# eps696/aphantasia

Measured on NVIDIA H100. Metric: optimization steps/sec @1280x720 FFT, 200 samples, ViT-B/32, higher is better.
Workload: dtype bf16

## Files before the change

aphantasia_b200/csrc/tc_gemm.cuh:

```cuda
#pragma once
#include "aph_common.cuh"
#include <cuda.h>

namespace aph {

typedef __nv_bfloat16 bf16;

struct GemmEpi {
  const float* bias = nullptr;
  const float* resid = nullptr;
  const bf16* gelu_in = nullptr;
  float* out_f32 = nullptr;
  bf16* out_bf16 = nullptr;
  bf16* out_pre = nullptr;
  int act = 0;
  int unpatch_p = 0;
  int unpatch_g = 0;
  int ld_resid = 0;
  int ld_out = 0;
};

struct GemmShape { int M, N, K; };

constexpr int GEMM_BM = 128;
constexpr int GEMM_BK = 64;
constexpr int GEMM_UK = 16;
constexpr int GEMM_THREADS = 3 * 128;

enum : int {
  EPI_F32 = 0,
  EPI_BF16 = 1,
  EPI_BIAS_BF16 = 2,
  EPI_BIAS_GELU = 3,
  EPI_BIAS_RESID = 4,
  EPI_GELUGRAD_BF16 = 5,
  EPI_UNPATCH = 6,
  EPI_KINDS = 7
};

__device__ __forceinline__ uint32_t smem_u32(const void* p) { return (uint32_t)__cvta_generic_to_shared(p); }

__device__ __forceinline__ void mbar_init(uint64_t* bar, uint32_t count) {
  asm volatile("mbarrier.init.shared::cta.b64 [%0], %1;" ::"r"(smem_u32(bar)), "r"(count));
}
__device__ __forceinline__ void mbar_expect_tx(uint64_t* bar, uint32_t bytes) {
  asm volatile("mbarrier.arrive.expect_tx.shared::cta.b64 _, [%0], %1;" ::"r"(smem_u32(bar)), "r"(bytes) : "memory");
}
__device__ __forceinline__ void mbar_arrive(uint64_t* bar) {
  asm volatile("mbarrier.arrive.shared::cta.b64 _, [%0];" ::"r"(smem_u32(bar)) : "memory");
}
__device__ __forceinline__ void mbar_wait(uint64_t* bar, uint32_t parity) {
  uint32_t done;
  do {
    asm volatile(
        "{\n\t.reg .pred p;\n\t"
        "mbarrier.try_wait.parity.shared::cta.b64 p, [%1], %2;\n\t"
        "selp.u32 %0, 1, 0, p;\n\t}"
        : "=r"(done) : "r"(smem_u32(bar)), "r"(parity) : "memory");
  } while (!done);
}
__device__ __forceinline__ void fence_barrier_init() { asm volatile("fence.mbarrier_init.release.cluster;" ::: "memory"); }

__device__ __forceinline__ void tma_prefetch_desc(const CUtensorMap* m) {
  asm volatile("prefetch.tensormap [%0];" ::"l"(reinterpret_cast<uint64_t>(m)) : "memory");
}
__device__ __forceinline__ void tma_load_2d(void* dst, const CUtensorMap* m, uint64_t* bar, int x, int y) {
  asm volatile("cp.async.bulk.tensor.2d.shared::cluster.global.mbarrier::complete_tx::bytes [%0], [%1, {%3, %4}], [%2];"
               ::"r"(smem_u32(dst)), "l"(reinterpret_cast<uint64_t>(m)), "r"(smem_u32(bar)), "r"(x), "r"(y) : "memory");
}
__device__ __forceinline__ void tma_load_3d(uint32_t dst_saddr, const CUtensorMap* m, uint64_t* bar, int x, int y, int z) {
  asm volatile("cp.async.bulk.tensor.3d.shared::cluster.global.mbarrier::complete_tx::bytes [%0], [%1, {%3, %4, %5}], [%2];"
               ::"r"(dst_saddr), "l"(reinterpret_cast<uint64_t>(m)), "r"(smem_u32(bar)), "r"(x), "r"(y), "r"(z) : "memory");
}
__device__ __forceinline__ void tma_load_2d_hint(void* dst, const CUtensorMap* m, uint64_t* bar, int x, int y, uint64_t policy) {
  asm volatile("cp.async.bulk.tensor.2d.shared::cluster.global.mbarrier::complete_tx::bytes.L2::cache_hint [%0], [%1, {%3, %4}], [%2], %5;"
               ::"r"(smem_u32(dst)), "l"(reinterpret_cast<uint64_t>(m)), "r"(smem_u32(bar)), "r"(x), "r"(y), "l"(policy) : "memory");
}
__device__ __forceinline__ uint64_t l2_policy_evict_last() {
  uint64_t p;
  asm volatile("createpolicy.fractional.L2::evict_last.b64 %0, 1.0;" : "=l"(p));
  return p;
}

__device__ __forceinline__ uint64_t make_smem_desc(uint32_t saddr) {
  uint64_t d = 0;
  d |= (uint64_t)((saddr & 0x3FFFF) >> 4);
  d |= (uint64_t)1 << 16;
  d |= (uint64_t)(1024 >> 4) << 32;
  d |= (uint64_t)1 << 62;
  return d;
}
__device__ __forceinline__ void wgmma_fence() { asm volatile("wgmma.fence.sync.aligned;" ::: "memory"); }
__device__ __forceinline__ void wgmma_commit() { asm volatile("wgmma.commit_group.sync.aligned;" ::: "memory"); }
template <int N> __device__ __forceinline__ void wgmma_wait() { asm volatile("wgmma.wait_group.sync.aligned %0;" ::"n"(N) : "memory"); }
template <int R> __device__ __forceinline__ void setmaxnreg_inc() { asm volatile("setmaxnreg.inc.sync.aligned.u32 %0;" ::"n"(R)); }
template <int R> __device__ __forceinline__ void setmaxnreg_dec() { asm volatile("setmaxnreg.dec.sync.aligned.u32 %0;" ::"n"(R)); }

template <int BN> struct Wgmma;
#define APH_WG_REGS8(o) "+f"(d[o]), "+f"(d[o + 1]), "+f"(d[o + 2]), "+f"(d[o + 3]), "+f"(d[o + 4]), "+f"(d[o + 5]), "+f"(d[o + 6]), "+f"(d[o + 7])
template <> struct Wgmma<128> {
  static __device__ __forceinline__ void mma(float (&d)[64], uint64_t da, uint64_t db, int acc) {
    asm volatile(
        "{\n\t.reg .pred p;\n\tsetp.ne.b32 p, %66, 0;\n\t"
        "wgmma.mma_async.sync.aligned.m64n128k16.f32.bf16.bf16 "
        "{%0, %1, %2, %3, %4, %5, %6, %7, %8, %9, %10, %11, %12, %13, %14, %15, %16, %17, %18, %19, %20, %21, %22, %23, "
        "%24, %25, %26, %27, %28, %29, %30, %31, %32, %33, %34, %35, %36, %37, %38, %39, %40, %41, %42, %43, %44, %45, %46, %47, "
        "%48, %49, %50, %51, %52, %53, %54, %55, %56, %57, %58, %59, %60, %61, %62, %63}, %64, %65, p, 1, 1, 0, 0;\n\t}"
        : APH_WG_REGS8(0), APH_WG_REGS8(8), APH_WG_REGS8(16), APH_WG_REGS8(24), APH_WG_REGS8(32), APH_WG_REGS8(40), APH_WG_REGS8(48), APH_WG_REGS8(56)
        : "l"(da), "l"(db), "r"(acc));
  }
};
template <> struct Wgmma<256> {
  static __device__ __forceinline__ void mma(float (&d)[128], uint64_t da, uint64_t db, int acc) {
    asm volatile(
        "{\n\t.reg .pred p;\n\tsetp.ne.b32 p, %130, 0;\n\t"
        "wgmma.mma_async.sync.aligned.m64n256k16.f32.bf16.bf16 "
        "{%0, %1, %2, %3, %4, %5, %6, %7, %8, %9, %10, %11, %12, %13, %14, %15, %16, %17, %18, %19, %20, %21, %22, %23, "
        "%24, %25, %26, %27, %28, %29, %30, %31, %32, %33, %34, %35, %36, %37, %38, %39, %40, %41, %42, %43, %44, %45, %46, %47, "
        "%48, %49, %50, %51, %52, %53, %54, %55, %56, %57, %58, %59, %60, %61, %62, %63, %64, %65, %66, %67, %68, %69, %70, %71, "
        "%72, %73, %74, %75, %76, %77, %78, %79, %80, %81, %82, %83, %84, %85, %86, %87, %88, %89, %90, %91, %92, %93, %94, %95, "
        "%96, %97, %98, %99, %100, %101, %102, %103, %104, %105, %106, %107, %108, %109, %110, %111, %112, %113, %114, %115, "
        "%116, %117, %118, %119, %120, %121, %122, %123, %124, %125, %126, %127}, %128, %129, p, 1, 1, 0, 0;\n\t}"
        : APH_WG_REGS8(0), APH_WG_REGS8(8), APH_WG_REGS8(16), APH_WG_REGS8(24), APH_WG_REGS8(32), APH_WG_REGS8(40), APH_WG_REGS8(48), APH_WG_REGS8(56),
          APH_WG_REGS8(64), APH_WG_REGS8(72), APH_WG_REGS8(80), APH_WG_REGS8(88), APH_WG_REGS8(96), APH_WG_REGS8(104), APH_WG_REGS8(112), APH_WG_REGS8(120)
        : "l"(da), "l"(db), "r"(acc));
  }
};
#undef APH_WG_REGS8

__device__ __forceinline__ float sigmoid1702(float x) {
  float t;
  asm("tanh.approx.f32 %0, %1;" : "=f"(t) : "f"(0.851f * x));
  return fmaf(0.5f, t, 0.5f);
}
__device__ __forceinline__ float quickgelu(float x) { return x * sigmoid1702(x); }
__device__ __forceinline__ float quickgelu_grad(float x) {
  const float s = sigmoid1702(x);
  return s * (1.f + 1.702f * x * (1.f - s));
}
__device__ __forceinline__ uint32_t pack_bf16(float lo, float hi) {
  __nv_bfloat162 v = __floats2bfloat162_rn(lo, hi);
  return *reinterpret_cast<uint32_t*>(&v);
}

template <int BN>
struct GemmCfg {
  static constexpr int A_BYTES = GEMM_BM * GEMM_BK * 2;
  static constexpr int B_BYTES = BN * GEMM_BK * 2;
  static constexpr int STAGE_BYTES = A_BYTES + B_BYTES;
  static constexpr int STAGES = (BN == 256) ? 4 : 6;
  static constexpr int BAR_OFFSET = STAGES * STAGE_BYTES;
  static constexpr int SMEM = BAR_OFFSET + 2 * STAGES * 8 + 1024;
};

__device__ __forceinline__ void consumer_bar_sync(int id) { asm volatile("bar.sync %0, 256;" ::"r"(id) : "memory"); }
__device__ __forceinline__ void consumer_bar_arrive(int id) { asm volatile("bar.arrive %0, 256;" ::"r"(id) : "memory"); }

template <int EPI>
constexpr bool epi_bf16_out() { return EPI == EPI_BF16 || EPI == EPI_BIAS_BF16 || EPI == EPI_BIAS_GELU || EPI == EPI_GELUGRAD_BF16; }

template <int EPI>
__device__ __forceinline__ void epi_store2(const GemmEpi& epi, size_t out_row, size_t res_row, int row, int col, float v0, float v1,
                                           float2 bb) {
  const size_t off = out_row + col;
  if (EPI == EPI_F32) {
    *reinterpret_cast<float2*>(epi.out_f32 + off) = make_float2(v0, v1);
  } else if (EPI == EPI_BIAS_RESID) {
    const float2 r = __ldg(reinterpret_cast<const float2*>(epi.resid + res_row + col));
    *reinterpret_cast<float2*>(epi.out_f32 + off) = make_float2(v0 + bb.x + r.x, v1 + bb.y + r.y);
  } else {
    const int p = epi.unpatch_p, g = epi.unpatch_g, R = p * g;
    const int ch = col / (p * p), rem = col - ch * p * p, py = rem / p, px = rem - py * p;
    const int s = row / (g * g), pr = row - s * g * g, gy = pr / g, gx = pr - gy * g;
    *reinterpret_cast<float2*>(epi.out_f32 + (((size_t)s * 3 + ch) * R + gy * p + py) * R + gx * p + px) = make_float2(v0, v1);
  }
}

__device__ __forceinline__ void st_global_16(void* p, const uint32_t (&w)[4]) {
  asm volatile("st.global.v4.b32 [%0], {%1, %2, %3, %4};" ::"l"(p), "r"(w[0]), "r"(w[1]), "r"(w[2]), "r"(w[3]) : "memory");
}

__device__ __forceinline__ void quad_transpose(uint32_t (&w)[4], int q) {
  const bool b0 = q & 1, b1 = q & 2;
#pragma unroll
  for (int p = 0; p < 2; ++p) {
    const uint32_t r = __shfl_xor_sync(0xffffffffu, b0 ? w[2 * p] : w[2 * p + 1], 1);
    if (b0) w[2 * p] = r; else w[2 * p + 1] = r;
  }
#pragma unroll
  for (int p = 0; p < 2; ++p) {
    const uint32_t r = __shfl_xor_sync(0xffffffffu, b1 ? w[p] : w[p + 2], 2);
    if (b1) w[p] = r; else w[p + 2] = r;
  }
}

template <int EPI>
__device__ __forceinline__ void epi_store_bf16x32(const GemmEpi& epi, int row, bool valid, int col0, int q, const float* v,
                                                  const float2* bb) {
  const size_t off = (size_t)row * epi.ld_out + col0 + 8 * q;
  uint32_t w[4], w2[4];
  if constexpr (EPI == EPI_GELUGRAD_BF16) {
    uint4 g = make_uint4(0u, 0u, 0u, 0u);
    if (valid) g = __ldg(reinterpret_cast<const uint4*>(epi.gelu_in + off));
    w2[0] = g.x; w2[1] = g.y; w2[2] = g.z; w2[3] = g.w;
    quad_transpose(w2, q);
  }
#pragma unroll
  for (int t = 0; t < 4; ++t) {
    float v0 = v[2 * t], v1 = v[2 * t + 1];
    if (EPI == EPI_BF16) {
      w[t] = pack_bf16(v0, v1);
    } else if (EPI == EPI_BIAS_BF16) {
      w[t] = pack_bf16(v0 + bb[t].x, v1 + bb[t].y);
    } else if (EPI == EPI_BIAS_GELU) {
      v0 += bb[t].x; v1 += bb[t].y;
      w2[t] = pack_bf16(v0, v1);
      w[t] = pack_bf16(quickgelu(v0), quickgelu(v1));
    } else {
      const float2 h = __bfloat1622float2(*reinterpret_cast<const __nv_bfloat162*>(&w2[t]));
      w[t] = pack_bf16(v0 * quickgelu_grad(h.x), v1 * quickgelu_grad(h.y));
    }
  }
  quad_transpose(w, q);
  if (valid) st_global_16(epi.out_bf16 + off, w);
  if constexpr (EPI == EPI_BIAS_GELU) {
    quad_transpose(w2, q);
    if (valid) st_global_16(epi.out_pre + off, w2);
  }
}

template <int BN, bool PINGPONG, int EPI>
__global__ void __launch_bounds__(GEMM_THREADS, 1)
k_gemm_bf16_tn(const __grid_constant__ CUtensorMap map_a, const __grid_constant__ CUtensorMap map_b, GemmShape shp, GemmEpi epi) {
  static_assert(BN == 128 || !PINGPONG, "the ping-pong schedule runs 128 x 128 tiles");
  using L = GemmCfg<BN>;
  constexpr int STAGES = L::STAGES;
  constexpr int MMAS = PINGPONG ? 2 : 1;
  constexpr bool HAS_BIAS = (EPI == EPI_BIAS_BF16 || EPI == EPI_BIAS_GELU || EPI == EPI_BIAS_RESID);
  pdl_trigger();
  extern __shared__ uint8_t smem_raw[];
  uint8_t* smem = reinterpret_cast<uint8_t*>((reinterpret_cast<uintptr_t>(smem_raw) + 1023) & ~(uintptr_t)1023);
  uint64_t* full_bar = reinterpret_cast<uint64_t*>(smem + L::BAR_OFFSET);
  uint64_t* empty_bar = full_bar + STAGES;

  const int wg = threadIdx.x >> 7, tid = threadIdx.x & 127;
  const int m_tiles = (shp.M + GEMM_BM - 1) / GEMM_BM, n_tiles = shp.N / BN;
  const int num_tiles = m_tiles * n_tiles, k_blocks = shp.K / GEMM_BK;

  if (threadIdx.x == 0) {
    tma_prefetch_desc(&map_a); tma_prefetch_desc(&map_b);
    for (int i = 0; i < STAGES; ++i) { mbar_init(&full_bar[i], 1); mbar_init(&empty_bar[i], PINGPONG ? 1 : 2); }
    fence_barrier_init();
  }
  __syncthreads();
  pdl_wait();

  if (wg == 0) {
    setmaxnreg_dec<40>();
    if (tid == 0) {
      const uint64_t pol_b = l2_policy_evict_last();
      uint32_t it = 0;
      for (int tile = blockIdx.x; tile < num_tiles; tile += gridDim.x) {
        const int m_blk = tile / n_tiles, n_blk = tile - m_blk * n_tiles;
        for (int kb = 0; kb < k_blocks; ++kb, ++it) {
          const uint32_t s = it % STAGES, ph = (it / STAGES) & 1;
          mbar_wait(&empty_bar[s], ph ^ 1);
          uint8_t* sa = smem + s * L::STAGE_BYTES;
          mbar_expect_tx(&full_bar[s], L::STAGE_BYTES);
          tma_load_2d(sa, &map_a, &full_bar[s], kb * GEMM_BK, m_blk * GEMM_BM);
          tma_load_2d_hint(sa + L::A_BYTES, &map_b, &full_bar[s], kb * GEMM_BK, n_blk * BN, pol_b);
        }
      }
    }
  } else {
    setmaxnreg_inc<232>();
    const int c = wg - 1, warp = tid >> 5, lane = tid & 31;
    const int row_in_tile = (PINGPONG ? 0 : 64 * c) + 16 * warp + (lane >> 2), col_in_tile = 2 * (lane & 3);
    uint32_t it = PINGPONG ? c * k_blocks : 0;
    const int tile_step = (PINGPONG ? 2 : 1) * gridDim.x;
    for (int tile = blockIdx.x + (PINGPONG ? c * gridDim.x : 0); tile / n_tiles * GEMM_BM < shp.M; tile += tile_step) {
      if (PINGPONG && tile != (int)blockIdx.x) consumer_bar_sync(1 + c);
      float d[MMAS][BN / 2];
#pragma unroll
      for (int h = 0; h < MMAS; ++h)
#pragma unroll
        for (int r = 0; r < BN / 2; ++r) d[h][r] = 0.f;
      for (int kb = 0; kb < k_blocks; ++kb, ++it) {
        const uint32_t s = it % STAGES, ph = (it / STAGES) & 1;
        mbar_wait(&full_bar[s], ph);
        const uint64_t ds = make_smem_desc(smem_u32(smem + s * L::STAGE_BYTES));
        wgmma_fence();
#pragma unroll
        for (int k = 0; k < GEMM_BK / GEMM_UK; ++k)
#pragma unroll
          for (int h = 0; h < MMAS; ++h)
            Wgmma<BN>::mma(d[h], ds + (uint64_t)((PINGPONG ? h : c) * 512 + 2 * k), ds + (uint64_t)(L::A_BYTES / 16 + 2 * k), (kb | k) != 0);
        wgmma_commit();
        wgmma_wait<1>();
        if (kb > 0 && tid == 0) mbar_arrive(&empty_bar[(it - 1) % STAGES]);
      }
      if (PINGPONG && (tile + (int)gridDim.x) / n_tiles * GEMM_BM < shp.M) consumer_bar_arrive(1 + (c ^ 1));
      wgmma_wait<0>();
      if (tid == 0) mbar_arrive(&empty_bar[(it - 1) % STAGES]);
      if (PINGPONG) it += k_blocks;
      const int m_blk = tile / n_tiles, n_blk = tile - m_blk * n_tiles;
#pragma unroll
      for (int h = 0; h < MMAS; ++h) {
        const int row0 = m_blk * GEMM_BM + 64 * h + row_in_tile, row1 = row0 + 8;
        if constexpr (epi_bf16_out<EPI>()) {
#pragma unroll
          for (int j0 = 0; j0 < BN / 8; j0 += 4) {
            const int col0 = n_blk * BN + 8 * j0;
            float2 bb[4];
            float v0[8], v1[8];
#pragma unroll
            for (int t = 0; t < 4; ++t) {
              bb[t] = HAS_BIAS ? __ldg(reinterpret_cast<const float2*>(epi.bias + col0 + 8 * t + col_in_tile)) : make_float2(0.f, 0.f);
              v0[2 * t] = d[h][4 * (j0 + t)]; v0[2 * t + 1] = d[h][4 * (j0 + t) + 1];
              v1[2 * t] = d[h][4 * (j0 + t) + 2]; v1[2 * t + 1] = d[h][4 * (j0 + t) + 3];
            }
            epi_store_bf16x32<EPI>(epi, row0, row0 < shp.M, col0, lane & 3, v0, bb);
            epi_store_bf16x32<EPI>(epi, row1, row1 < shp.M, col0, lane & 3, v1, bb);
          }
        } else {
          const size_t out0 = (size_t)row0 * epi.ld_out, out1 = out0 + 8 * (size_t)epi.ld_out;
          const size_t res0 = (EPI == EPI_BIAS_RESID) ? (size_t)row0 * epi.ld_resid : 0, res1 = res0 + 8 * (size_t)epi.ld_resid;
#pragma unroll
          for (int j = 0; j < BN / 8; ++j) {
            const int col = n_blk * BN + 8 * j + col_in_tile;
            const float2 bb = HAS_BIAS ? __ldg(reinterpret_cast<const float2*>(epi.bias + col)) : make_float2(0.f, 0.f);
            if (row0 < shp.M) epi_store2<EPI>(epi, out0, res0, row0, col, d[h][4 * j], d[h][4 * j + 1], bb);
            if (row1 < shp.M) epi_store2<EPI>(epi, out1, res1, row1, col, d[h][4 * j + 2], d[h][4 * j + 3], bb);
          }
        }
      }
    }
  }
}

int make_tmap_bf16(CUtensorMap* out, const void* base, int rows, int K, int box_rows, int64_t row_stride = 0);
int make_tmap_bf16_tokens(CUtensorMap* out, const void* base, int cols, int T, int S, int box_rows);
int launch_gemm(const void* A, const void* B, GemmShape shp, const GemmEpi& epi, cudaStream_t st, int lda = 0);

}
```

aphantasia_b200/csrc/vit_gemm.cu:

```cuda
#include "tc_gemm.cuh"
#include <atomic>
#include <mutex>
#include <vector>
#include <utility>

namespace aph {

typedef CUresult (*EncodeTiledFn)(CUtensorMap*, CUtensorMapDataType, cuuint32_t, void*, const cuuint64_t*, const cuuint64_t*,
                                  const cuuint32_t*, const cuuint32_t*, CUtensorMapInterleave, CUtensorMapSwizzle,
                                  CUtensorMapL2promotion, CUtensorMapFloatOOBfill);

static EncodeTiledFn get_encode() {
  static EncodeTiledFn fn = nullptr;
  static std::once_flag once;
  std::call_once(once, [] {
    void* p = nullptr;
    cudaDriverEntryPointQueryResult q;
    if (cudaGetDriverEntryPoint("cuTensorMapEncodeTiled", &p, cudaEnableDefault, &q) == cudaSuccess && q == cudaDriverEntryPointSuccess)
      fn = reinterpret_cast<EncodeTiledFn>(p);
  });
  return fn;
}

int make_tmap_bf16(CUtensorMap* out, const void* base, int rows, int K, int box_rows, int64_t row_stride) {
  EncodeTiledFn enc = get_encode();
  APH_REQUIRE(enc != nullptr, "cuTensorMapEncodeTiled not available from the driver");
  if (row_stride == 0) row_stride = K;
  APH_REQUIRE(row_stride >= K, "tensor map: row stride %lld < K=%d", (long long)row_stride, K);
  APH_REQUIRE((reinterpret_cast<uintptr_t>(base) & 15) == 0 && row_stride % 8 == 0, "tensor map: base/stride not 16-byte aligned");
  const cuuint64_t gdim[2] = {(cuuint64_t)K, (cuuint64_t)rows};
  const cuuint64_t gstride[1] = {(cuuint64_t)row_stride * 2};
  const cuuint32_t box[2] = {(cuuint32_t)GEMM_BK, (cuuint32_t)box_rows};
  const cuuint32_t estr[2] = {1, 1};
  const CUresult r = enc(out, CU_TENSOR_MAP_DATA_TYPE_BFLOAT16, 2, const_cast<void*>(base), gdim, gstride, box, estr,
                         CU_TENSOR_MAP_INTERLEAVE_NONE, CU_TENSOR_MAP_SWIZZLE_128B, CU_TENSOR_MAP_L2_PROMOTION_L2_256B,
                         CU_TENSOR_MAP_FLOAT_OOB_FILL_NONE);
  APH_REQUIRE(r == CUDA_SUCCESS, "cuTensorMapEncodeTiled failed: CUresult %d (rows=%d K=%d box_rows=%d)", (int)r, rows, K, box_rows);
  return 0;
}

int make_tmap_bf16_tokens(CUtensorMap* out, const void* base, int cols, int T, int S, int box_rows) {
  EncodeTiledFn enc = get_encode();
  APH_REQUIRE(enc != nullptr, "cuTensorMapEncodeTiled not available from the driver");
  APH_REQUIRE((reinterpret_cast<uintptr_t>(base) & 15) == 0 && cols % 8 == 0, "tensor map: base/stride not 16-byte aligned");
  const cuuint64_t gdim[3] = {(cuuint64_t)cols, (cuuint64_t)T, (cuuint64_t)S};
  const cuuint64_t gstride[2] = {(cuuint64_t)cols * 2, (cuuint64_t)T * cols * 2};
  const cuuint32_t box[3] = {64u, (cuuint32_t)box_rows, 1u};
  const cuuint32_t estr[3] = {1, 1, 1};
  const CUresult r = enc(out, CU_TENSOR_MAP_DATA_TYPE_BFLOAT16, 3, const_cast<void*>(base), gdim, gstride, box, estr,
                         CU_TENSOR_MAP_INTERLEAVE_NONE, CU_TENSOR_MAP_SWIZZLE_128B, CU_TENSOR_MAP_L2_PROMOTION_L2_256B,
                         CU_TENSOR_MAP_FLOAT_OOB_FILL_NONE);
  APH_REQUIRE(r == CUDA_SUCCESS, "cuTensorMapEncodeTiled (tokens) failed: CUresult %d (cols=%d T=%d S=%d box_rows=%d)", (int)r, cols, T, S, box_rows);
  return 0;
}

static bool g_prof = false;
bool gemm_profiling_on() { return g_prof; }
static std::vector<std::pair<cudaEvent_t, cudaEvent_t>> g_prof_ev;
static std::vector<double> g_prof_flops;

static std::atomic<long long> g_variant_launches[2][EPI_KINDS];

template <int BN, bool PINGPONG, int EPI>
static int launch_cfg(const void* A, const void* B, GemmShape shp, const GemmEpi& epi, cudaStream_t st, int lda) {
  using L = GemmCfg<BN>;
  static_assert(L::SMEM <= 227 * 1024, "GEMM shared-memory budget");
  g_variant_launches[(PINGPONG || BN == 256) ? 1 : 0][EPI].fetch_add(1, std::memory_order_relaxed);
  static bool configured = false;
  if (!configured) {
    APH_CUDA_OK(cudaFuncSetAttribute(k_gemm_bf16_tn<BN, PINGPONG, EPI>, cudaFuncAttributeMaxDynamicSharedMemorySize, L::SMEM));
    configured = true;
  }
  CUtensorMap ma, mb;
  if (int e = make_tmap_bf16(&ma, A, shp.M, shp.K, GEMM_BM, lda)) return e;
  if (int e = make_tmap_bf16(&mb, B, shp.N, shp.K, BN)) return e;
  const int tiles = ((shp.M + GEMM_BM - 1) / GEMM_BM) * (shp.N / BN);
  const int grid = tiles < num_sms() ? tiles : num_sms();
  cudaEvent_t e0 = nullptr, e1 = nullptr;
  if (g_prof) { cudaEventCreate(&e0); cudaEventCreate(&e1); cudaEventRecord(e0, st); }
  APH_CUDA_OK(launch_k(k_gemm_bf16_tn<BN, PINGPONG, EPI>, dim3(grid), dim3(GEMM_THREADS), (size_t)L::SMEM, st, 1, ma, mb, shp, epi));
  APH_LAUNCH_OK();
  if (g_prof) { cudaEventRecord(e1, st); g_prof_ev.emplace_back(e0, e1); g_prof_flops.push_back(2.0 * shp.M * shp.N * shp.K); }
  return 0;
}

int launch_gemm(const void* A, const void* B, GemmShape shp, const GemmEpi& epi_in, cudaStream_t st, int lda) {
  APH_REQUIRE(A && B && shp.M > 0, "gemm: null operand or empty M");
  APH_REQUIRE(shp.K % GEMM_BK == 0 && shp.K > 0, "gemm: K=%d must be a positive multiple of %d", shp.K, GEMM_BK);
  APH_REQUIRE(shp.N % 128 == 0 && shp.N > 0, "gemm: N=%d must be a positive multiple of 128", shp.N);
  APH_REQUIRE(lda == 0 || lda >= shp.K, "gemm: lda=%d < K=%d", lda, shp.K);
  APH_REQUIRE((epi_in.ld_out == 0 || epi_in.ld_out >= shp.N) && (epi_in.ld_resid == 0 || epi_in.ld_resid >= shp.N),
              "gemm: output / residual row stride below N=%d", shp.N);
  GemmEpi epi = epi_in;
  if (epi.ld_out == 0) epi.ld_out = shp.N;
  if (epi.ld_resid == 0) epi.ld_resid = shp.N;
  int kind = -1;
  const bool b = epi.bias, r = epi.resid, gi = epi.gelu_in, f = epi.out_f32, h = epi.out_bf16, pre = epi.out_pre, act = epi.act == 1, un = epi.unpatch_p > 0;
  APH_REQUIRE(!un || epi.ld_out == shp.N, "gemm: the un-patchify store takes no output stride");
  if (un && f && !b && !r && !gi && !h && !pre && !act) kind = EPI_UNPATCH;
  else if (f && !h && !b && !r && !gi && !pre && !act) kind = EPI_F32;
  else if (h && !f && !b && !r && !gi && !pre && !act) kind = EPI_BF16;
  else if (h && !f && b && !r && !gi && !pre && !act) kind = EPI_BIAS_BF16;
  else if (h && !f && b && !r && !gi && pre && act) kind = EPI_BIAS_GELU;
  else if (f && !h && b && r && !gi && !pre && !act) kind = EPI_BIAS_RESID;
  else if (h && !f && !b && !r && gi && !pre && !act) kind = EPI_GELUGRAD_BF16;
  APH_REQUIRE(kind >= 0, "gemm: unsupported epilogue combination");
  const uintptr_t bf16_ptrs = reinterpret_cast<uintptr_t>(epi.out_bf16) | reinterpret_cast<uintptr_t>(epi.out_pre) | reinterpret_cast<uintptr_t>(epi.gelu_in);
  APH_REQUIRE((bf16_ptrs & 15) == 0 && ((size_t)epi.ld_out * (f ? 4 : 2)) % 16 == 0 && ((size_t)epi.ld_resid * 4) % 16 == 0 &&
              ((size_t)lda * 2) % 16 == 0,
              "gemm: bf16 epilogue operands and row strides must be 16-byte aligned (8 columns are stored per lane)");
  const int m_tiles = (shp.M + GEMM_BM - 1) / GEMM_BM;
  const bool pingpong = m_tiles * (shp.N / 128) >= 2 * num_sms() && shp.K <= 1024;
  const bool wide = !pingpong && shp.N % 256 == 0 && m_tiles * (shp.N / 256) >= num_sms();
#define APH_GEMM_CASE(K) case K: return pingpong ? launch_cfg<128, true, K>(A, B, shp, epi, st, lda) \
                                                 : wide ? launch_cfg<256, false, K>(A, B, shp, epi, st, lda) : launch_cfg<128, false, K>(A, B, shp, epi, st, lda);
  switch (kind) {
    APH_GEMM_CASE(EPI_F32) APH_GEMM_CASE(EPI_BF16) APH_GEMM_CASE(EPI_BIAS_BF16) APH_GEMM_CASE(EPI_BIAS_GELU)
    APH_GEMM_CASE(EPI_BIAS_RESID) APH_GEMM_CASE(EPI_GELUGRAD_BF16) APH_GEMM_CASE(EPI_UNPATCH)
  }
#undef APH_GEMM_CASE
  return 2;
}

}

using namespace aph;

extern "C" int aph_gemm_bf16_tn(const void* A, const void* B, float* C, int M, int N, int K, void* stream) {
  APH_REQUIRE(C != nullptr, "aph_gemm_bf16_tn: null output");
  GemmEpi epi;
  epi.out_f32 = C;
  return launch_gemm(A, B, GemmShape{M, N, K}, epi, (cudaStream_t)stream);
}

extern "C" int aph_gemm_epi_test(const void* A, const void* B, int M, int N, int K, const float* bias, const float* resid,
                                 const void* gelu_in, int act, float* out_f32, void* out_bf16, void* out_pre,
                                 int unpatch_p, int unpatch_g, void* stream) {
  GemmEpi epi;
  epi.bias = bias; epi.resid = resid; epi.gelu_in = reinterpret_cast<const bf16*>(gelu_in); epi.act = act;
  epi.out_f32 = out_f32; epi.out_bf16 = reinterpret_cast<bf16*>(out_bf16); epi.out_pre = reinterpret_cast<bf16*>(out_pre);
  epi.unpatch_p = unpatch_p; epi.unpatch_g = unpatch_g;
  return launch_gemm(A, B, GemmShape{M, N, K}, epi, (cudaStream_t)stream);
}

extern "C" int aph_gemm_epi_strided_test(const void* A, int lda, const void* B, int M, int N, int K, const float* bias,
                                         const float* resid, int ld_resid, const void* gelu_in, int act, float* out_f32,
                                         void* out_bf16, void* out_pre, int ld_out, void* stream) {
  GemmEpi epi;
  epi.bias = bias; epi.resid = resid; epi.gelu_in = reinterpret_cast<const bf16*>(gelu_in); epi.act = act;
  epi.out_f32 = out_f32; epi.out_bf16 = reinterpret_cast<bf16*>(out_bf16); epi.out_pre = reinterpret_cast<bf16*>(out_pre);
  epi.ld_resid = ld_resid; epi.ld_out = ld_out;
  return launch_gemm(A, B, GemmShape{M, N, K}, epi, (cudaStream_t)stream, lda);
}

extern "C" int64_t aph_gemm_variant_launches(int variant, int epi) {
  if (variant < 0 || variant > 1 || epi >= EPI_KINDS) return -1;
  long long n = 0;
  for (int k = 0; k < EPI_KINDS; ++k) if (epi < 0 || epi == k) n += g_variant_launches[variant][k].load();
  return (int64_t)n;
}

extern "C" int aph_prof_gemm(int enable, double* total_ms, double* total_flops, int* launches) {
  if (enable) { g_prof = true; g_prof_ev.clear(); g_prof_flops.clear(); return 0; }
  g_prof = false;
  double ms = 0., fl = 0.;
  for (size_t i = 0; i < g_prof_ev.size(); ++i) {
    APH_CUDA_OK(cudaEventSynchronize(g_prof_ev[i].second));
    float t = 0.f;
    APH_CUDA_OK(cudaEventElapsedTime(&t, g_prof_ev[i].first, g_prof_ev[i].second));
    ms += t; fl += g_prof_flops[i];
    cudaEventDestroy(g_prof_ev[i].first); cudaEventDestroy(g_prof_ev[i].second);
  }
  if (total_ms) *total_ms = ms;
  if (total_flops) *total_flops = fl;
  if (launches) *launches = (int)g_prof_ev.size();
  g_prof_ev.clear(); g_prof_flops.clear();
  return 0;
}
```

Before: 83.68.

## Stream residual and GELU-grad epilogue operands through TMA slabs in shared memory

For the bias+residual and GELU-gradient epilogues, the GEMM now has producer threads TMA-load the residual or GELU input into a ring of 128B-swizzled shared-memory slabs. Consumers combine those slabs with the accumulators in place, and the results are written back with TMA bulk stores. This replaces per-thread scattered global loads and stores in the epilogue with bulk asynchronous transfers that can overlap the mainloop. In exchange it takes one pipeline stage away from the mainloop to make room for the slabs, and it adds mbarrier and bulk-group synchronisation per slab.

```diff
diff --git a/aphantasia_b200/csrc/tc_gemm.cuh b/aphantasia_b200/csrc/tc_gemm.cuh
--- a/aphantasia_b200/csrc/tc_gemm.cuh
+++ b/aphantasia_b200/csrc/tc_gemm.cuh
@@ -76,6 +76,14 @@
   asm volatile("cp.async.bulk.tensor.2d.shared::cluster.global.mbarrier::complete_tx::bytes.L2::cache_hint [%0], [%1, {%3, %4}], [%2], %5;"
                ::"r"(smem_u32(dst)), "l"(reinterpret_cast<uint64_t>(m)), "r"(smem_u32(bar)), "r"(x), "r"(y), "l"(policy) : "memory");
 }
+__device__ __forceinline__ void tma_store_2d(const CUtensorMap* m, const void* src, int x, int y) {
+  asm volatile("cp.async.bulk.tensor.2d.global.shared::cta.bulk_group [%0, {%2, %3}], [%1];"
+               ::"l"(reinterpret_cast<uint64_t>(m)), "r"(smem_u32(src)), "r"(x), "r"(y) : "memory");
+}
+__device__ __forceinline__ void bulk_commit() { asm volatile("cp.async.bulk.commit_group;" ::: "memory"); }
+template <int N> __device__ __forceinline__ void bulk_wait_read() { asm volatile("cp.async.bulk.wait_group.read %0;" ::"n"(N) : "memory"); }
+__device__ __forceinline__ void bulk_wait_all() { asm volatile("cp.async.bulk.wait_group 0;" ::: "memory"); }
+__device__ __forceinline__ void fence_proxy_async_smem() { asm volatile("fence.proxy.async.shared::cta;" ::: "memory"); }
 __device__ __forceinline__ uint64_t l2_policy_evict_last() {
   uint64_t p;
   asm volatile("createpolicy.fractional.L2::evict_last.b64 %0, 1.0;" : "=l"(p));
@@ -143,31 +151,36 @@
   return *reinterpret_cast<uint32_t*>(&v);
 }
 
-template <int BN>
+template <int EPI>
+constexpr bool epi_tma() { return EPI == EPI_BIAS_RESID || EPI == EPI_GELUGRAD_BF16; }
+
+template <int BN, int EPI>
 struct GemmCfg {
   static constexpr int A_BYTES = GEMM_BM * GEMM_BK * 2;
   static constexpr int B_BYTES = BN * GEMM_BK * 2;
   static constexpr int STAGE_BYTES = A_BYTES + B_BYTES;
-  static constexpr int STAGES = (BN == 256) ? 4 : 6;
-  static constexpr int BAR_OFFSET = STAGES * STAGE_BYTES;
-  static constexpr int SMEM = BAR_OFFSET + 2 * STAGES * 8 + 1024;
+  static constexpr bool TMA_EPI = epi_tma<EPI>();
+  static constexpr int STAGES = TMA_EPI ? (BN == 256 ? 3 : 5) : (BN == 256 ? 4 : 6);
+  static constexpr int SLAB_BYTES = 64 * 128;
+  static constexpr int SLAB_COLS = (EPI == EPI_BIAS_RESID) ? 32 : 64;
+  static constexpr int SLABS = TMA_EPI ? (BN == 256 ? 5 : 4) : 0;
+  static constexpr int SLAB_OFFSET = STAGES * STAGE_BYTES;
+  static constexpr int BAR_OFFSET = SLAB_OFFSET + 2 * SLABS * SLAB_BYTES;
+  static constexpr int SMEM = BAR_OFFSET + 2 * STAGES * 8 + 4 * SLABS * 8 + 1024;
 };
 
 __device__ __forceinline__ void consumer_bar_sync(int id) { asm volatile("bar.sync %0, 256;" ::"r"(id) : "memory"); }
 __device__ __forceinline__ void consumer_bar_arrive(int id) { asm volatile("bar.arrive %0, 256;" ::"r"(id) : "memory"); }
+__device__ __forceinline__ void wg_bar_sync(int id) { asm volatile("bar.sync %0, 128;" ::"r"(id) : "memory"); }
 
 template <int EPI>
-constexpr bool epi_bf16_out() { return EPI == EPI_BF16 || EPI == EPI_BIAS_BF16 || EPI == EPI_BIAS_GELU || EPI == EPI_GELUGRAD_BF16; }
+constexpr bool epi_bf16_out() { return EPI == EPI_BF16 || EPI == EPI_BIAS_BF16 || EPI == EPI_BIAS_GELU; }
 
 template <int EPI>
-__device__ __forceinline__ void epi_store2(const GemmEpi& epi, size_t out_row, size_t res_row, int row, int col, float v0, float v1,
-                                           float2 bb) {
+__device__ __forceinline__ void epi_store2(const GemmEpi& epi, size_t out_row, int row, int col, float v0, float v1) {
   const size_t off = out_row + col;
   if (EPI == EPI_F32) {
     *reinterpret_cast<float2*>(epi.out_f32 + off) = make_float2(v0, v1);
-  } else if (EPI == EPI_BIAS_RESID) {
-    const float2 r = __ldg(reinterpret_cast<const float2*>(epi.resid + res_row + col));
-    *reinterpret_cast<float2*>(epi.out_f32 + off) = make_float2(v0 + bb.x + r.x, v1 + bb.y + r.y);
   } else {
     const int p = epi.unpatch_p, g = epi.unpatch_g, R = p * g;
     const int ch = col / (p * p), rem = col - ch * p * p, py = rem / p, px = rem - py * p;
@@ -199,12 +212,6 @@
                                                   const float2* bb) {
   const size_t off = (size_t)row * epi.ld_out + col0 + 8 * q;
   uint32_t w[4], w2[4];
-  if constexpr (EPI == EPI_GELUGRAD_BF16) {
-    uint4 g = make_uint4(0u, 0u, 0u, 0u);
-    if (valid) g = __ldg(reinterpret_cast<const uint4*>(epi.gelu_in + off));
-    w2[0] = g.x; w2[1] = g.y; w2[2] = g.z; w2[3] = g.w;
-    quad_transpose(w2, q);
-  }
 #pragma unroll
   for (int t = 0; t < 4; ++t) {
     float v0 = v[2 * t], v1 = v[2 * t + 1];
@@ -212,13 +219,10 @@
       w[t] = pack_bf16(v0, v1);
     } else if (EPI == EPI_BIAS_BF16) {
       w[t] = pack_bf16(v0 + bb[t].x, v1 + bb[t].y);
-    } else if (EPI == EPI_BIAS_GELU) {
+    } else {
       v0 += bb[t].x; v1 += bb[t].y;
       w2[t] = pack_bf16(v0, v1);
       w[t] = pack_bf16(quickgelu(v0), quickgelu(v1));
-    } else {
-      const float2 h = __bfloat1622float2(*reinterpret_cast<const __nv_bfloat162*>(&w2[t]));
-      w[t] = pack_bf16(v0 * quickgelu_grad(h.x), v1 * quickgelu_grad(h.y));
     }
   }
   quad_transpose(w, q);
@@ -229,12 +233,57 @@
   }
 }
 
+__device__ __forceinline__ int swz128(int r, int k) { return r * 128 + ((k ^ (r & 7)) << 4); }
+
+__device__ __forceinline__ float2 lds_f2(uint32_t a) {
+  float2 v;
+  asm volatile("ld.shared.v2.f32 {%0, %1}, [%2];" : "=f"(v.x), "=f"(v.y) : "r"(a) : "memory");
+  return v;
+}
+__device__ __forceinline__ void sts_f2(uint32_t a, float2 v) { asm volatile("st.shared.v2.f32 [%0], {%1, %2};" ::"r"(a), "f"(v.x), "f"(v.y) : "memory"); }
+__device__ __forceinline__ uint32_t lds_u32(uint32_t a) {
+  uint32_t v;
+  asm volatile("ld.shared.b32 %0, [%1];" : "=r"(v) : "r"(a) : "memory");
+  return v;
+}
+__device__ __forceinline__ void sts_u32(uint32_t a, uint32_t v) { asm volatile("st.shared.b32 [%0], %1;" ::"r"(a), "r"(v) : "memory"); }
+__device__ __forceinline__ float2 bf16x2_to_float2(uint32_t w) { return __bfloat1622float2(*reinterpret_cast<const __nv_bfloat162*>(&w)); }
+
+template <int EPI, int NACC>
+__device__ __forceinline__ void epi_slab(uint32_t slab, const float (&v)[NACC], int g0, int rs, int q, const float* bias_cols) {
+  if constexpr (EPI == EPI_BIAS_RESID) {
+    const bool odd = rs & 1;
+#pragma unroll
+    for (int t = 0; t < 4; ++t) {
+      const int g = t ^ (odd ? 2 : 0);
+      const int a = 4 * (g0 + t), b = 4 * (g0 + (t ^ 2));
+      const float a0 = odd ? v[b] : v[a], a1 = odd ? v[b + 1] : v[a + 1];
+      const float a2 = odd ? v[b + 2] : v[a + 2], a3 = odd ? v[b + 3] : v[a + 3];
+      const float2 bb = __ldg(reinterpret_cast<const float2*>(bias_cols + 8 * g + 2 * q));
+      const uint32_t p0 = slab + swz128(rs, 2 * g + (q >> 1)) + 8 * (q & 1), p1 = slab + swz128(rs + 8, 2 * g + (q >> 1)) + 8 * (q & 1);
+      const float2 r0 = lds_f2(p0), r1 = lds_f2(p1);
+      sts_f2(p0, make_float2(a0 + bb.x + r0.x, a1 + bb.y + r0.y));
+      sts_f2(p1, make_float2(a2 + bb.x + r1.x, a3 + bb.y + r1.y));
+    }
+  } else {
+#pragma unroll
+    for (int t = 0; t < 8; ++t) {
+      const int a = 4 * (g0 + t);
+      const uint32_t p0 = slab + swz128(rs, t) + 4 * q, p1 = slab + swz128(rs + 8, t) + 4 * q;
+      const float2 h0 = bf16x2_to_float2(lds_u32(p0)), h1 = bf16x2_to_float2(lds_u32(p1));
+      sts_u32(p0, pack_bf16(v[a] * quickgelu_grad(h0.x), v[a + 1] * quickgelu_grad(h0.y)));
+      sts_u32(p1, pack_bf16(v[a + 2] * quickgelu_grad(h1.x), v[a + 3] * quickgelu_grad(h1.y)));
+    }
+  }
+}
+
 template <int BN, bool PINGPONG, int EPI>
 __global__ void __launch_bounds__(GEMM_THREADS, 1)
-k_gemm_bf16_tn(const __grid_constant__ CUtensorMap map_a, const __grid_constant__ CUtensorMap map_b, GemmShape shp, GemmEpi epi) {
+k_gemm_bf16_tn(const __grid_constant__ CUtensorMap map_a, const __grid_constant__ CUtensorMap map_b, GemmShape shp, GemmEpi epi,
+               const __grid_constant__ CUtensorMap map_ei, const __grid_constant__ CUtensorMap map_eo) {
   static_assert(BN == 128 || !PINGPONG, "the ping-pong schedule runs 128 x 128 tiles");
-  using L = GemmCfg<BN>;
-  constexpr int STAGES = L::STAGES;
+  using L = GemmCfg<BN, EPI>;
+  constexpr int STAGES = L::STAGES, SLABS = L::SLABS;
   constexpr int MMAS = PINGPONG ? 2 : 1;
   constexpr bool HAS_BIAS = (EPI == EPI_BIAS_BF16 || EPI == EPI_BIAS_GELU || EPI == EPI_BIAS_RESID);
   pdl_trigger();
@@ -242,6 +291,8 @@
   uint8_t* smem = reinterpret_cast<uint8_t*>((reinterpret_cast<uintptr_t>(smem_raw) + 1023) & ~(uintptr_t)1023);
   uint64_t* full_bar = reinterpret_cast<uint64_t*>(smem + L::BAR_OFFSET);
   uint64_t* empty_bar = full_bar + STAGES;
+  uint64_t* slab_full = empty_bar + STAGES;
+  uint64_t* slab_empty = slab_full + 2 * SLABS;
 
   const int wg = threadIdx.x >> 7, tid = threadIdx.x & 127;
   const int m_tiles = (shp.M + GEMM_BM - 1) / GEMM_BM, n_tiles = shp.N / BN;
@@ -249,7 +300,9 @@
 
   if (threadIdx.x == 0) {
     tma_prefetch_desc(&map_a); tma_prefetch_desc(&map_b);
+    if constexpr (SLABS > 0) { tma_prefetch_desc(&map_ei); tma_prefetch_desc(&map_eo); }
     for (int i = 0; i < STAGES; ++i) { mbar_init(&full_bar[i], 1); mbar_init(&empty_bar[i], PINGPONG ? 1 : 2); }
+    for (int i = 0; i < 2 * SLABS; ++i) { mbar_init(&slab_full[i], 1); mbar_init(&slab_empty[i], 1); }
     fence_barrier_init();
   }
   __syncthreads();
@@ -257,6 +310,22 @@
 
   if (wg == 0) {
     setmaxnreg_dec<40>();
+    if constexpr (SLABS > 0) if (tid == 32 || tid == 64) {
+      const int r = (tid >> 5) - 1;
+      uint8_t* ring = smem + L::SLAB_OFFSET + r * SLABS * L::SLAB_BYTES;
+      uint32_t sit = 0;
+      for (int tile = blockIdx.x + (PINGPONG ? r * gridDim.x : 0); tile < num_tiles; tile += (PINGPONG ? 2 : 1) * gridDim.x) {
+        const int m_blk = tile / n_tiles, n_blk = tile - m_blk * n_tiles;
+        for (int h = 0; h < MMAS; ++h)
+          for (int j = 0; j < BN / L::SLAB_COLS; ++j, ++sit) {
+            const uint32_t s = sit % SLABS, ph = (sit / SLABS) & 1;
+            mbar_wait(&slab_empty[r * SLABS + s], ph ^ 1);
+            mbar_expect_tx(&slab_full[r * SLABS + s], L::SLAB_BYTES);
+            tma_load_2d(ring + s * L::SLAB_BYTES, &map_ei, &slab_full[r * SLABS + s], n_blk * BN + j * L::SLAB_COLS,
+                        m_blk * GEMM_BM + 64 * (PINGPONG ? h : r));
+          }
+      }
+    }
     if (tid == 0) {
       const uint64_t pol_b = l2_policy_evict_last();
       uint32_t it = 0;
@@ -277,6 +346,7 @@
     const int c = wg - 1, warp = tid >> 5, lane = tid & 31;
     const int row_in_tile = (PINGPONG ? 0 : 64 * c) + 16 * warp + (lane >> 2), col_in_tile = 2 * (lane & 3);
     uint32_t it = PINGPONG ? c * k_blocks : 0;
+    [[maybe_unused]] uint32_t sit = 0;
     const int tile_step = (PINGPONG ? 2 : 1) * gridDim.x;
     for (int tile = blockIdx.x + (PINGPONG ? c * gridDim.x : 0); tile / n_tiles * GEMM_BM < shp.M; tile += tile_step) {
       if (PINGPONG && tile != (int)blockIdx.x) consumer_bar_sync(1 + c);
@@ -304,37 +374,65 @@
       if (tid == 0) mbar_arrive(&empty_bar[(it - 1) % STAGES]);
       if (PINGPONG) it += k_blocks;
       const int m_blk = tile / n_tiles, n_blk = tile - m_blk * n_tiles;
-#pragma unroll
-      for (int h = 0; h < MMAS; ++h) {
-        const int row0 = m_blk * GEMM_BM + 64 * h + row_in_tile, row1 = row0 + 8;
-        if constexpr (epi_bf16_out<EPI>()) {
-#pragma unroll
-          for (int j0 = 0; j0 < BN / 8; j0 += 4) {
-            const int col0 = n_blk * BN + 8 * j0;
-            float2 bb[4];
-            float v0[8], v1[8];
-#pragma unroll
-            for (int t = 0; t < 4; ++t) {
-              bb[t] = HAS_BIAS ? __ldg(reinterpret_cast<const float2*>(epi.bias + col0 + 8 * t + col_in_tile)) : make_float2(0.f, 0.f);
-              v0[2 * t] = d[h][4 * (j0 + t)]; v0[2 * t + 1] = d[h][4 * (j0 + t) + 1];
-              v1[2 * t] = d[h][4 * (j0 + t) + 2]; v1[2 * t + 1] = d[h][4 * (j0 + t) + 3];
+      if constexpr (SLABS > 0) {
+        uint8_t* ring = smem + L::SLAB_OFFSET + c * SLABS * L::SLAB_BYTES;
+        const int rs = 16 * warp + (lane >> 2), q = lane & 3;
+#pragma unroll
+        for (int h = 0; h < MMAS; ++h) {
+#pragma unroll
+          for (int j = 0; j < BN / L::SLAB_COLS; ++j, ++sit) {
+            const uint32_t s = sit % SLABS;
+            uint8_t* slab = ring + s * L::SLAB_BYTES;
+            mbar_wait(&slab_full[c * SLABS + s], (sit / SLABS) & 1);
+            epi_slab<EPI>(smem_u32(slab), d[h], j * L::SLAB_COLS / 8, rs, q, HAS_BIAS ? epi.bias + n_blk * BN + j * L::SLAB_COLS : nullptr);
+            fence_proxy_async_smem();
+            wg_bar_sync(3 + c);
+            if (tid == 0) {
+              tma_store_2d(&map_eo, slab, n_blk * BN + j * L::SLAB_COLS, m_blk * GEMM_BM + 64 * (PINGPONG ? h : c));
+              bulk_commit();
+              if (h > 0 || j > 0) {
+                bulk_wait_read<1>();
+                mbar_arrive(&slab_empty[c * SLABS + (sit - 1) % SLABS]);
+              }
             }
-            epi_store_bf16x32<EPI>(epi, row0, row0 < shp.M, col0, lane & 3, v0, bb);
-            epi_store_bf16x32<EPI>(epi, row1, row1 < shp.M, col0, lane & 3, v1, bb);
           }
-        } else {
-          const size_t out0 = (size_t)row0 * epi.ld_out, out1 = out0 + 8 * (size_t)epi.ld_out;
-          const size_t res0 = (EPI == EPI_BIAS_RESID) ? (size_t)row0 * epi.ld_resid : 0, res1 = res0 + 8 * (size_t)epi.ld_resid;
-#pragma unroll
-          for (int j = 0; j < BN / 8; ++j) {
-            const int col = n_blk * BN + 8 * j + col_in_tile;
-            const float2 bb = HAS_BIAS ? __ldg(reinterpret_cast<const float2*>(epi.bias + col)) : make_float2(0.f, 0.f);
-            if (row0 < shp.M) epi_store2<EPI>(epi, out0, res0, row0, col, d[h][4 * j], d[h][4 * j + 1], bb);
-            if (row1 < shp.M) epi_store2<EPI>(epi, out1, res1, row1, col, d[h][4 * j + 2], d[h][4 * j + 3], bb);
+        }
+        if (tid == 0) {
+          bulk_wait_read<0>();
+          mbar_arrive(&slab_empty[c * SLABS + (sit - 1) % SLABS]);
+        }
+      } else {
+#pragma unroll
+        for (int h = 0; h < MMAS; ++h) {
+          const int row0 = m_blk * GEMM_BM + 64 * h + row_in_tile, row1 = row0 + 8;
+          if constexpr (epi_bf16_out<EPI>()) {
+#pragma unroll
+            for (int j0 = 0; j0 < BN / 8; j0 += 4) {
+              const int col0 = n_blk * BN + 8 * j0;
+              float2 bb[4];
+              float v0[8], v1[8];
+#pragma unroll
+              for (int t = 0; t < 4; ++t) {
+                bb[t] = HAS_BIAS ? __ldg(reinterpret_cast<const float2*>(epi.bias + col0 + 8 * t + col_in_tile)) : make_float2(0.f, 0.f);
+                v0[2 * t] = d[h][4 * (j0 + t)]; v0[2 * t + 1] = d[h][4 * (j0 + t) + 1];
+                v1[2 * t] = d[h][4 * (j0 + t) + 2]; v1[2 * t + 1] = d[h][4 * (j0 + t) + 3];
+              }
+              epi_store_bf16x32<EPI>(epi, row0, row0 < shp.M, col0, lane & 3, v0, bb);
+              epi_store_bf16x32<EPI>(epi, row1, row1 < shp.M, col0, lane & 3, v1, bb);
+            }
+          } else {
+            const size_t out0 = (size_t)row0 * epi.ld_out, out1 = out0 + 8 * (size_t)epi.ld_out;
+#pragma unroll
+            for (int j = 0; j < BN / 8; ++j) {
+              const int col = n_blk * BN + 8 * j + col_in_tile;
+              if (row0 < shp.M) epi_store2<EPI>(epi, out0, row0, col, d[h][4 * j], d[h][4 * j + 1]);
+              if (row1 < shp.M) epi_store2<EPI>(epi, out1, row1, col, d[h][4 * j + 2], d[h][4 * j + 3]);
+            }
           }
         }
       }
     }
+    if constexpr (SLABS > 0) if (tid == 0) bulk_wait_all();
   }
 }
 
diff --git a/aphantasia_b200/csrc/vit_gemm.cu b/aphantasia_b200/csrc/vit_gemm.cu
--- a/aphantasia_b200/csrc/vit_gemm.cu
+++ b/aphantasia_b200/csrc/vit_gemm.cu
@@ -61,9 +61,27 @@
 
 static std::atomic<long long> g_variant_launches[2][EPI_KINDS];
 
+static int make_tmap_slab(CUtensorMap* out, const void* base, bool f32, int rows, int cols, int row_stride) {
+  EncodeTiledFn enc = get_encode();
+  APH_REQUIRE(enc != nullptr, "cuTensorMapEncodeTiled not available from the driver");
+  const int esz = f32 ? 4 : 2;
+  APH_REQUIRE((reinterpret_cast<uintptr_t>(base) & 15) == 0 && ((size_t)row_stride * esz) % 16 == 0,
+              "gemm: the residual / gelu input and the output must be 16-byte aligned, with 16-byte aligned row strides");
+  const cuuint64_t gdim[2] = {(cuuint64_t)cols, (cuuint64_t)rows};
+  const cuuint64_t gstride[1] = {(cuuint64_t)row_stride * esz};
+  const cuuint32_t box[2] = {(cuuint32_t)(128 / esz), 64u};
+  const cuuint32_t estr[2] = {1, 1};
+  const CUresult r = enc(out, f32 ? CU_TENSOR_MAP_DATA_TYPE_FLOAT32 : CU_TENSOR_MAP_DATA_TYPE_BFLOAT16, 2, const_cast<void*>(base), gdim,
+                         gstride, box, estr, CU_TENSOR_MAP_INTERLEAVE_NONE, CU_TENSOR_MAP_SWIZZLE_128B, CU_TENSOR_MAP_L2_PROMOTION_L2_256B,
+                         CU_TENSOR_MAP_FLOAT_OOB_FILL_NONE);
+  APH_REQUIRE(r == CUDA_SUCCESS, "cuTensorMapEncodeTiled (epilogue slab) failed: CUresult %d (rows=%d cols=%d stride=%d)", (int)r, rows,
+              cols, row_stride);
+  return 0;
+}
+
 template <int BN, bool PINGPONG, int EPI>
 static int launch_cfg(const void* A, const void* B, GemmShape shp, const GemmEpi& epi, cudaStream_t st, int lda) {
-  using L = GemmCfg<BN>;
+  using L = GemmCfg<BN, EPI>;
   static_assert(L::SMEM <= 227 * 1024, "GEMM shared-memory budget");
   g_variant_launches[(PINGPONG || BN == 256) ? 1 : 0][EPI].fetch_add(1, std::memory_order_relaxed);
   static bool configured = false;
@@ -71,14 +89,21 @@
     APH_CUDA_OK(cudaFuncSetAttribute(k_gemm_bf16_tn<BN, PINGPONG, EPI>, cudaFuncAttributeMaxDynamicSharedMemorySize, L::SMEM));
     configured = true;
   }
-  CUtensorMap ma, mb;
+  CUtensorMap ma, mb, mei = {}, meo = {};
   if (int e = make_tmap_bf16(&ma, A, shp.M, shp.K, GEMM_BM, lda)) return e;
   if (int e = make_tmap_bf16(&mb, B, shp.N, shp.K, BN)) return e;
+  if constexpr (EPI == EPI_BIAS_RESID) {
+    if (int e = make_tmap_slab(&mei, epi.resid, true, shp.M, shp.N, epi.ld_resid)) return e;
+    if (int e = make_tmap_slab(&meo, epi.out_f32, true, shp.M, shp.N, epi.ld_out)) return e;
+  } else if constexpr (EPI == EPI_GELUGRAD_BF16) {
+    if (int e = make_tmap_slab(&mei, epi.gelu_in, false, shp.M, shp.N, epi.ld_out)) return e;
+    if (int e = make_tmap_slab(&meo, epi.out_bf16, false, shp.M, shp.N, epi.ld_out)) return e;
+  }
   const int tiles = ((shp.M + GEMM_BM - 1) / GEMM_BM) * (shp.N / BN);
   const int grid = tiles < num_sms() ? tiles : num_sms();
   cudaEvent_t e0 = nullptr, e1 = nullptr;
   if (g_prof) { cudaEventCreate(&e0); cudaEventCreate(&e1); cudaEventRecord(e0, st); }
-  APH_CUDA_OK(launch_k(k_gemm_bf16_tn<BN, PINGPONG, EPI>, dim3(grid), dim3(GEMM_THREADS), (size_t)L::SMEM, st, 1, ma, mb, shp, epi));
+  APH_CUDA_OK(launch_k(k_gemm_bf16_tn<BN, PINGPONG, EPI>, dim3(grid), dim3(GEMM_THREADS), (size_t)L::SMEM, st, 1, ma, mb, shp, epi, mei, meo));
   APH_LAUNCH_OK();
   if (g_prof) { cudaEventRecord(e1, st); g_prof_ev.emplace_back(e0, e1); g_prof_flops.push_back(2.0 * shp.M * shp.N * shp.K); }
   return 0;
```

Result: no change. 84.29 (median of 6 runs) (+0.7%).
